# bluenote-1577/sylph

Hardware: AMD Instinct MI355X
Metric: read Gbp/s sketched + genome-comparisons/s profiled, 1 Gbp vs GTDB-R220 (higher is better)
Workload: dtype u64

## Files before the change

sylph_amd/csrc/reads.hip:

```cpp
#include <cstddef>

#include "common.h"
#include "device_common.h"
#include "reads_block.h"
#include "seed_plan.h"
#include "sketch_session.h"

namespace sylph {

namespace {

__global__ __launch_bounds__(256) void block_records_kernel(const uint64_t* __restrict__ off, uint64_t n_rec, uint32_t bias,
                                                            uint32_t rt, uint32_t n_entries, uint32_t* __restrict__ blk_rec,
                                                            uint32_t* __restrict__ count_sentinel, uint32_t* __restrict__ state_words) {
    const uint32_t b = blockIdx.x * blockDim.x + threadIdx.x;
    if (b == 0) { *count_sentinel = 0; state_words[0] = 0; state_words[1] = 0; }
    if (b >= n_entries) return;
    blk_rec[b] = (uint32_t)first_record_of_block(off, n_rec, bias, b, rt);
}

#ifndef SYLPH_READS_HASH_DEFAULT
#define SYLPH_READS_HASH_DEFAULT 1
#endif
#ifndef SYLPH_READS_WAVES
#define SYLPH_READS_WAVES 5
#endif
template <int K, int HV, int ENC, int TPB>
__global__ __launch_bounds__(TPB) __attribute__((amdgpu_waves_per_eu(TPB == 256 ? SYLPH_READS_WAVES : 6, TPB == 256 ? SYLPH_READS_WAVES : 6))) void reads_kernel(const uint8_t* __restrict__ bases_al, uint32_t bias, uint64_t n_al,
                                                     const uint64_t* __restrict__ off, uint64_t n_rec,
                                                     const uint32_t* __restrict__ blk_rec, uint32_t n_blk, uint32_t it_begin, uint32_t it_end,
                                                     uint32_t rt, uint64_t thr,
                                                     uint32_t cand_slack, int avx2_compat, int paired, int want_markers, uint64_t rec_base,
                                                     uint32_t slot_cap, OccRec* __restrict__ slot_rec,
                                                     uint32_t* __restrict__ slot_key, int key_sh,
                                                     uint32_t* __restrict__ blk_count,
                                                     ReadsState* __restrict__ state, const uint32_t* __restrict__ blk_list,
                                                     uint32_t* __restrict__ spill_slot_of_blk) {
    const ReadsLds<TPB> s = reads_lds<TPB>();
    const uint32_t tid = threadIdx.x;
    const uint64_t thr_loop = HV == 2 ? (uint64_t)((uint32_t)(thr >> 32) + 1u + cand_slack) : thr;
    if (tid == 0) *s.redo = 0;
    const uint32_t n_words = stream_words(rt), per_xcd = xcd_share(n_blk);
    for (uint32_t it0 = it_begin + blockIdx.x; it0 < it_end; it0 += gridDim.x) {
        const uint32_t it = blk_list ? it0 : xcd_deal_share(it0, per_xcd);
        if (it >= n_blk) continue;
        const uint32_t blk = blk_list ? blk_list[it] : it;
        const int64_t a0 = block_a0(blk, rt);
        load_stream<ENC, TPB>(s.sF, bases_al, n_al, a0, n_words);
        const uint64_t R0 = blk_rec[blk], R1 = blk_rec[blk + 1];
        const uint64_t w_lo = paired ? (R0 & ~1ull) : R0;
        const bool in_lds = stage_offsets(s, off, n_rec, R0, R1, w_lo);
        __syncthreads();
        uint32_t base_prev = 0;
        const uint64_t out0 = (uint64_t)it * slot_cap;
        for (uint64_t pass = R0; pass < R1; pass += TPB) {
            uint64_t L, s1, s2, e2;
            uint32_t nh, rel;
            if (record_geometry<K>(s, off, in_lds, w_lo, pass + tid, R1, paired, bias, a0, avx2_compat, L, s1, s2, e2, nh, rel))
                state->long_record = 1u;
            uint32_t slot, rel_h, nh_h, rows;
            const bool dealt = deal_by_length(s, nh, rel, slot, rel_h, nh_h, rows);
            hash_record<K, HV>(s, slot, rel_h, nh_h, thr_loop);
            if (dealt) __syncthreads();
            uint32_t total = 0;
            for (;;) {
                uint32_t first;
                const uint32_t cnt = count_hits(s, nh, first, total);
                publish_markers(s, cnt, first, total, want_markers, paired, L, s1, s2, e2, rel, bias, a0);
                const bool is_listed = list_survivors(s, nh, cnt, first, total, rows);
                __syncthreads();
                finish_survivors<K, HV>(s, is_listed, rows, total, base_prev, slot_cap, thr, rec_base, pass, paired, avx2_compat, out0, slot_rec,
                                        slot_key, key_sh);
                __syncthreads();
                if constexpr (HV != 2) break;
                else {
                    if (!*s.redo) break;
                    __syncthreads();
                    if (tid == 0) *s.redo = 0;
                }
            }
            base_prev += total;
        }
        if (tid == 0) close_slots(blk_list != nullptr, blk, it, base_prev, slot_cap, blk_count, &state->spill, spill_slot_of_blk);
        __syncthreads();
    }
}

__global__ __launch_bounds__(64) void compact_occ_kernel(const OccRec* __restrict__ slot_rec, const uint32_t* __restrict__ blk_count,
                                                         const uint32_t* __restrict__ blk_off, uint32_t n_blk, uint32_t slot_cap,
                                                         uint32_t spill_cap, const OccRec* __restrict__ spill_rec,
                                                         const uint32_t* __restrict__ spill_slot_of_blk,
                                                         uint64_t* __restrict__ out_hash, OccRec* __restrict__ out_rec) {
    for (uint32_t b = blockIdx.x; b < n_blk; b += gridDim.x) {
        const uint32_t n = blk_count[b], d = blk_off[b];
        const OccRec* sr = slot_rec + (uint64_t)b * slot_cap;
        if (n > slot_cap) sr = spill_rec + (uint64_t)spill_slot_of_blk[b] * spill_cap;
        for (uint32_t i = threadIdx.x; i < n; i += blockDim.x) {
            const OccRec r = sr[i];
            out_hash[d + i] = r.hash;
            out_rec[d + i] = r;
        }
    }
}

uint32_t grid_for(uint64_t n, uint32_t tpb = 256) { return (uint32_t)((n + tpb - 1) / tpb); }

__global__ __launch_bounds__(1024) void block_total_kernel(const uint32_t* __restrict__ blk_count, uint32_t n_blk, uint32_t* __restrict__ total) {
    __shared__ uint32_t s[16];
    uint32_t v = 0;
    for (uint32_t i = threadIdx.x; i < n_blk; i += 1024) v += blk_count[i];
#pragma unroll
    for (int d = 32; d > 0; d >>= 1) v += (uint32_t)__shfl_xor((int)v, d);
    if ((threadIdx.x & 63) == 0) s[threadIdx.x >> 6] = v;
    __syncthreads();
    if (threadIdx.x == 0) {
        uint32_t t = 0;
        for (int w = 0; w < 16; w++) t += s[w];
        *total = t;
    }
}

void compact_region(sylph_sketch* sk, uint32_t n_blk, uint32_t slot_cap, uint32_t n, uint32_t spill_cap, const OccRec* spill_rec) {
    sylph_ctx* ctx = sk->ctx;
    const SlotMeta m = slot_meta_of(sk, n_blk);
    exclusive_sum_u32(ctx, m.blk_count, m.blk_off, (size_t)n_blk + 1);
    const uint64_t need = sk->n_occ + n;
    sk->hash.grow_keep(need * 8, sk->n_occ * 8, ctx->stream);
    sk->recs.grow_keep(need * sizeof(OccRec), sk->n_occ * sizeof(OccRec), ctx->stream);
    {
        ScopedKernelTimer t(ctx, "compact");
        hipLaunchKernelGGL(compact_occ_kernel, dim3(std::min<uint32_t>(n_blk, 1u << 16)), dim3(64), 0, ctx->stream,
                           sk->slot_rec.as<OccRec>(), m.blk_count, m.blk_off, n_blk, slot_cap, spill_cap, spill_rec, m.spill_slot,
                           sk->hash.as<uint64_t>() + sk->n_occ, sk->recs.as<OccRec>() + sk->n_occ);
        SY_HIP(hipGetLastError());
    }
    sk->n_occ = need;
}

}

void resolve_deferred_slots(sylph_sketch* sk) {
    if (!sk->pend.live || !sk->pend.deferred) return;
    sylph_ctx* ctx = sk->ctx;
    const SlotMeta m = slot_meta_of(sk, sk->pend.n_blk);
    hipLaunchKernelGGL(block_total_kernel, dim3(1), dim3(1024), 0, ctx->stream, m.blk_count, sk->pend.n_blk, m.blk_off + sk->pend.n_blk);
    uint32_t res[3] = {0, 0, 0};
    ctx->read_back(res, m.blk_off + sk->pend.n_blk, 12);
    if (res[1] || res[2]) { redo_deferred_batch(sk); return; }
    sk->pend.deferred = false;
    sk->pend.n = res[0];
    if (res[0] == 0) sk->pend = PendingSlots{};
}

void flush_pending_slots(sylph_sketch* sk) {
    resolve_deferred_slots(sk);
    if (!sk->pend.live) return;
    compact_region(sk, sk->pend.n_blk, sk->pend.slot_cap, sk->pend.n, 0, nullptr);
    sk->pend = PendingSlots{};
}

bool push_short_reads(sylph_sketch* sk, const uint8_t* d_bases, uint32_t phase, const uint64_t* d_off, uint64_t n_records, uint64_t n_bases,
                      int enc) {
    sylph_ctx* ctx = sk->ctx;
    const uint32_t bias = enc == SYLPH_ENC_2BIT ? (uint32_t)((uintptr_t)d_bases & 15) * 4u + phase : (uint32_t)((uintptr_t)d_bases & 15);
    const uint8_t* bases_al = d_bases - ((uintptr_t)d_bases & 15);
    const uint64_t n_al = n_bases + bias;
    static const int env_ragged_tpb = [] { const char* e = getenv("SYLPH_HIP_READS_RAGGED_TPB"); return e ? atoi(e) : RTPB; }();
    const ReadsBlockPlan plan = reads_block_plan(n_bases, n_records, bias, sk->c, sk->k, env_ragged_tpb == RTPB_RAGGED);
    const int tpb = plan.tpb;
    const uint32_t rt = plan.rt, n_blk = plan.n_blk, spill_cap = plan.spill_cap, slot_cap = plan.slot_cap;
    const size_t lds_bytes = plan.lds_bytes;
    const uint64_t thr = UINT64_MAX / (uint64_t)sk->c;
    sk->slot_rec.reserve((size_t)n_blk * slot_cap * sizeof(OccRec));
    sk->slot_key.reserve((size_t)n_blk * slot_cap * 4);
    sk->slot_meta.reserve(SlotMeta::bytes(n_blk, sizeof(ReadsState)));
    const SlotMeta m = slot_meta_of(sk, n_blk);
    ReadsState* const state = reinterpret_cast<ReadsState*>(m.state_words);
    static_assert(offsetof(ReadsState, long_record) == 0 && offsetof(ReadsState, spill) == 4 && offsetof(SpillState, n_tiles) == 0,
                  "long_record and spill.n_tiles are the first two words");
    int cus = 256;
    (void)hipDeviceGetAttribute(&cus, hipDeviceAttributeMultiprocessorCount, ctx->device);
    const int hv_want = ctx->reads_hash >= 0 ? ctx->reads_hash : hash_variant_env(SYLPH_READS_HASH_DEFAULT);
    const uint32_t slack = ctx->reads_slack;
    const int hv = (hv_want == 2 && ((thr >> 32) + 1ull + slack) > 0xFFFFFFFFull) ? 1 : hv_want;
    const int key_sh = key_shift(sk->c);
    auto launch = [&](uint32_t n_it, uint32_t it_b, uint32_t it_e, uint32_t cap, OccRec* sr, uint32_t* skey, const uint32_t* list) {
        if (it_e <= it_b) return;
        const uint32_t grid = ctx->reads_wg_per_cu ? (uint32_t)std::min<uint64_t>(it_e - it_b, (uint64_t)cus * ctx->reads_wg_per_cu) : it_e - it_b;
        auto go = [&](auto kc, auto hc, auto ec, auto tc) {
            constexpr int KK = decltype(kc)::value, HH = decltype(hc)::value, EE = decltype(ec)::value, TT = decltype(tc)::value;
            hipLaunchKernelGGL((reads_kernel<KK, HH, EE, TT>), dim3(grid), dim3(TT), lds_bytes, ctx->stream, bases_al, bias, n_al, d_off, n_records,
                               m.blk_rec, n_it, it_b, it_e, rt, thr, slack, sk->avx2_compat, sk->paired, sk->no_dedup ? 0 : 1, sk->rec_base, cap, sr, skey,
                               key_sh, m.blk_count, state, list, m.spill_slot);
        };
        auto with_tpb = [&](auto kc, auto hc, auto ec) {
            if (tpb == RTPB_RAGGED) go(kc, hc, ec, std::integral_constant<int, RTPB_RAGGED>{}); else go(kc, hc, ec, std::integral_constant<int, RTPB>{});
        };
        if (enc == SYLPH_ENC_2BIT) with_k_hv<1, 2>(sk->k, hv, [&](auto kc, auto hc) { with_tpb(kc, hc, std::integral_constant<int, 1>{}); });
        else with_k_hv<0, 2>(sk->k, hv, [&](auto kc, auto hc) { with_tpb(kc, hc, std::integral_constant<int, 0>{}); });
        SY_HIP(hipGetLastError());
    };
    {
        HostPhase ph(ctx, "push: reads kernel");
        {
            ScopedKernelTimer t(ctx, "annotate");
            hipLaunchKernelGGL(block_records_kernel, dim3(grid_for(n_blk + 1)), dim3(256), 0, ctx->stream, d_off, n_records, bias, rt,
                               n_blk + 1, m.blk_rec, m.blk_count + n_blk, m.state_words);
        }
        ctx->seed_gate();
        {
            const uint32_t n_round = xcd_positions(n_blk);
            const uint32_t cut = xcd_tail_cut(n_blk, ctx->turn.done && !ctx->turn.recorded ? ctx->reads_tail_pct : 0);
            {
                ScopedKernelTimer t(ctx, "seeds");
                launch(n_blk, 0, cut, slot_cap, sk->slot_rec.as<OccRec>(), sk->slot_key.as<uint32_t>(), nullptr);
            }
            ctx->seed_done();
            if (cut < n_round) {
                ScopedKernelTimer t(ctx, "seeds");
                launch(n_blk, cut, n_round, slot_cap, sk->slot_rec.as<OccRec>(), sk->slot_key.as<uint32_t>(), nullptr);
            }
        }
        const uint64_t n_expect = plan.n_expect;
        if (sk->borrow_until_finish && sk->n_occ == 0 && sk->rec_base == 0 && ctx->finish_mode == 0 && sk->c >= 2 && n_expect >= 4096 &&
            (uint64_t)n_blk * slot_cap < (1ull << 31)) {
            sk->pend = PendingSlots{};
            sk->pend.live = true;
            sk->pend.deferred = true;
            sk->pend.n_blk = n_blk;
            sk->pend.slot_cap = slot_cap;
            sk->pend.n = n_blk * slot_cap;
            sk->pend.n_expect = (uint32_t)std::min<uint64_t>(n_expect, sk->pend.n);
            sk->pend.bases = d_bases; sk->pend.phase = phase; sk->pend.off = d_off;
            sk->pend.n_records = n_records; sk->pend.n_bases = n_bases; sk->pend.enc = enc;
            if (ctx->profile) ctx->stats["deferred"].launches++;
            return true;
        }
        hipLaunchKernelGGL(block_total_kernel, dim3(1), dim3(1024), 0, ctx->stream, m.blk_count, n_blk, m.blk_off + n_blk);
    }
    uint32_t res[3] = {0, 0, 0};
    SY_HIP(hipMemcpyAsync(ctx->pinned, m.blk_off + n_blk, 12, hipMemcpyDeviceToHost, ctx->stream));
    SY_HIP(hipStreamSynchronize(ctx->stream));
    memcpy(res, ctx->pinned, 12);
    if (!ctx->pending.empty()) profile_collect(ctx);
    if (res[1] || res[2] > SPILL_MAX_TILES) return false;
    const uint32_t n = res[0];
    if (n == 0) return true;
    if (res[2] == 0 && sk->n_occ == 0 && ctx->finish_mode != 1 && sk->c >= 2) {
        sk->pend.live = true;
        sk->pend.n_blk = n_blk;
        sk->pend.slot_cap = slot_cap;
        sk->pend.n = n;
        return true;
    }
    const OccRec* sp_r = nullptr;
    if (res[2]) {
        DevBuf& b_x = ctx->scratch[7];
        b_x.reserve((size_t)res[2] * spill_cap * sizeof(OccRec));
        OccRec* xr = b_x.as<OccRec>();
        ScopedKernelTimer ts(ctx, "seeds_spill");
        ScopedKernelTimer t(ctx, "seeds");
        launch(res[2], 0, res[2], spill_cap, xr, nullptr, state->spill.tiles);
        sp_r = xr;
    }
    compact_region(sk, n_blk, slot_cap, n, spill_cap, sp_r);
    return true;
}

}
```

sylph_amd/csrc/reads_block.h:

```cpp
#pragma once
#include "common.h"
#include "device_common.h"
#include "seed_plan.h"
#include "sketch_session.h"

namespace sylph {
namespace {

using namespace seed_plan;

template <int K>
struct KC {
    static constexpr uint64_t MASK = (1ull << (2 * K)) - 1;
};

#define SY_LDS __attribute__((address_space(3)))
template <int TPB>
struct ReadsLds {
    SY_LDS uint32_t* sF;
    SY_LDS uint64_t* off;
    SY_LDS uint64_t *m0, *m1;
    SY_LDS uint32_t (*mask)[TPB];
    SY_LDS uint32_t* wave;
    SY_LDS uint32_t* first;
    SY_LDS uint32_t* hist;
    SY_LDS uint32_t* rel;
    SY_LDS uint16_t *perm, *nh;
    SY_LDS uint32_t *redo, *redo_deal;
};
template <int TPB>
__device__ __forceinline__ ReadsLds<TPB> reads_lds() {
    constexpr int OFFS = offs_staged(TPB);
    extern __shared__ uint32_t sF[];
    __shared__ uint64_t s_off[OFFS + 4];
    __shared__ uint32_t s_mask[MASKW][TPB];
    __shared__ uint32_t s_wave[TPB / 64];
    __shared__ uint32_t s_first[TPB + 1], s_rel[TPB];
    __shared__ uint16_t s_perm[TPB], s_nh[TPB];
    __shared__ uint32_t s_redo, s_redo_deal;
    static_assert((OFFS + 4) >= 2 * TPB, "the marker arrays alias the staged offsets");
    static_assert(TPB + 1 >= 64, "the histogram aliases s_first");
    using W = SY_LDS uint32_t*; using D = SY_LDS uint64_t*; using H = SY_LDS uint16_t*;
    return ReadsLds<TPB>{(W)sF, (D)s_off, (D)s_off, (D)s_off + TPB, (SY_LDS uint32_t(*)[TPB])s_mask, (W)s_wave, (W)s_first, (W)s_first, (W)s_rel,
                         (H)s_perm, (H)s_nh, (W)&s_redo, (W)&s_redo_deal};
}

__device__ __forceinline__ uint64_t win64(const SY_LDS uint32_t* sF, uint32_t b) {
    const uint32_t j = b >> 4, ph = (b & 15u) * 2u;
    const uint64_t x = ((uint64_t)sF[j] << 32) | sF[j + 1];
    return (x << ph) | ((uint64_t)sF[j + 2] >> (32u - ph));
}

template <int K>
__device__ __forceinline__ uint64_t revcomp_top(uint64_t x) {
    const uint64_t rev = __brevll(x);
    const uint64_t y = ((rev & 0x5555555555555555ull) << 1) | ((rev >> 1) & 0x5555555555555555ull);
    return (~y) & KC<K>::MASK;
}

__device__ __forceinline__ uint32_t even_fields_to_bytes31(uint32_t w) {
    uint32_t t = w & 0xCCCCCCCCu;
    t = (t | (t << 2)) & 0xF0F0F0F0u;
    return t | (t << 4);
}
__device__ __forceinline__ void evenodd16(uint64_t x, uint32_t& ev, uint32_t& od) {
    const uint32_t hi = (uint32_t)(x >> 32), lo = (uint32_t)x;
    ev = __builtin_amdgcn_perm(even_fields_to_bytes31(hi), even_fields_to_bytes31(lo), 0x07050301u);
    od = __builtin_amdgcn_perm(even_fields_to_bytes31(hi << 2), even_fields_to_bytes31(lo << 2), 0x07050301u);
}

template <int K, int T, int HV>
__device__ __forceinline__ void kmer_step(uint32_t A0, uint32_t A1, uint32_t A2, uint32_t B0, uint32_t B1, uint32_t B2,
                                          uint64_t thr, uint32_t& mask) {
    static_assert(2 * K <= 62 && 2 * K > 32, "min_u62 wants both windows below 2^62; the high word holds 2K - 32 bits");
    constexpr int HB = 2 * K - 32, T0 = T & ~1;
    uint32_t fhi, rhi;
    if constexpr (2 * T + HB <= 32) {
        fhi = __builtin_amdgcn_ubfe(A0, 32 - HB - 2 * T, HB); rhi = __builtin_amdgcn_ubfe(B1, 2 * T, HB);
    } else {
        const uint32_t cf = fword<2 * T0>(A0, A1, A2), cr = rword<2 * T0 + 32>(B0, B1, B2);
        fhi = __builtin_amdgcn_ubfe(cf, 32 - HB - 2 * (T - T0), HB); rhi = __builtin_amdgcn_ubfe(cr, 2 * (T - T0), HB);
    }
    const uint32_t flo = fword<2 * T + HB>(A0, A1, A2), rlo = rword<2 * T>(B0, B1, B2);
    const uint64_t canon = min_u62(((uint64_t)fhi << 32) | flo, ((uint64_t)rhi << 32) | rlo);
    if constexpr (HV == 2) {
        const uint32_t u = mm_hash64_gfx950_hi1(canon);
        asm("v_cmp_ge_u32 vcc, %2, %1\n\tv_addc_co_u32 %0, vcc, %0, %0, vcc" : "+v"(mask) : "v"(u), "s"((uint32_t)thr) : "vcc");
    } else {
        const uint64_t h = HV ? mm_hash64_gfx950(canon) : mm_hash64(canon);
        asm("v_cmp_lt_u64 vcc, %1, %2\n\tv_addc_co_u32 %0, vcc, %0, %0, vcc" : "+v"(mask) : "v"(h), "s"(thr) : "vcc");
    }
}
template <int K, int T0, int HV>
__device__ __forceinline__ void kmer_steps8(uint32_t A0, uint32_t A1, uint32_t A2, uint32_t B0, uint32_t B1, uint32_t B2,
                                            uint64_t thr, uint32_t& mask) {
    kmer_step<K, T0 + 0, HV>(A0, A1, A2, B0, B1, B2, thr, mask);
    kmer_step<K, T0 + 1, HV>(A0, A1, A2, B0, B1, B2, thr, mask);
    kmer_step<K, T0 + 2, HV>(A0, A1, A2, B0, B1, B2, thr, mask);
    kmer_step<K, T0 + 3, HV>(A0, A1, A2, B0, B1, B2, thr, mask);
    kmer_step<K, T0 + 4, HV>(A0, A1, A2, B0, B1, B2, thr, mask);
    kmer_step<K, T0 + 5, HV>(A0, A1, A2, B0, B1, B2, thr, mask);
    kmer_step<K, T0 + 6, HV>(A0, A1, A2, B0, B1, B2, thr, mask);
    kmer_step<K, T0 + 7, HV>(A0, A1, A2, B0, B1, B2, thr, mask);
}

template <int ENC, int TPB>
__device__ __forceinline__ void load_stream(SY_LDS uint32_t* sF, const uint8_t* bases_al, uint64_t n_al, int64_t a0, uint32_t n_words) {
    const uint32_t tid = threadIdx.x;
    const bool interior = a0 >= 0 && (uint64_t)(a0 + (int64_t)n_words * 16) <= n_al;
    if (interior) {
        if constexpr (ENC == 0) {
            const uint4* src = reinterpret_cast<const uint4*>(bases_al + a0);
            for (uint32_t ci = tid; ci < n_words; ci += TPB) sF[ci] = pack16_fwd(src[ci]);
        } else {
            const uint32_t* src = reinterpret_cast<const uint32_t*>(bases_al + (a0 >> 2));
            for (uint32_t ci = tid; ci < n_words; ci += TPB) sF[ci] = __builtin_amdgcn_perm(0u, src[ci], 0x00010203u);
        }
    } else {
        for (uint32_t ci = tid; ci < n_words; ci += TPB) {
            const int64_t a = a0 + (int64_t)ci * 16;
            if constexpr (ENC == 0) {
                uint4 v = make_uint4(0, 0, 0, 0);
                if (a >= 0 && (uint64_t)a < n_al) v = *reinterpret_cast<const uint4*>(bases_al + a);
                sF[ci] = pack16_fwd(v);
            } else {
                uint32_t w = 0;
                if (a >= 0 && (uint64_t)a < n_al) w = *reinterpret_cast<const uint32_t*>(bases_al + (a >> 2));
                sF[ci] = __builtin_amdgcn_perm(0u, w, 0x00010203u);
            }
        }
    }
}

template <int TPB>
__device__ __forceinline__ bool stage_offsets(const ReadsLds<TPB> s, const uint64_t* off, uint64_t n_rec, uint64_t R0, uint64_t R1,
                                              uint64_t w_lo) {
    const uint64_t w_hi = min(R1 + 2, n_rec);
    const bool in_lds = (w_hi - w_lo + 1) <= (uint64_t)(offs_staged(TPB) + 4) && (R1 - R0) <= (uint64_t)TPB;
    if (in_lds)
        for (uint64_t t = threadIdx.x; t <= w_hi - w_lo; t += TPB) s.off[t] = off[w_lo + t];
    return in_lds;
}

template <int K, int TPB>
__device__ __forceinline__ bool record_geometry(const ReadsLds<TPB> s, const uint64_t* off, bool in_lds, uint64_t w_lo, uint64_t r,
                                                uint64_t R1, int paired, uint32_t bias, int64_t a0, int avx2_compat, uint64_t& L,
                                                uint64_t& s1, uint64_t& s2, uint64_t& e2, uint32_t& nh, uint32_t& rel) {
    const bool active = r < R1;
    uint64_t start = 0;
    L = 0; s1 = 0; s2 = 0; e2 = 0;
    if (active) {
        if (in_lds) {
            start = s.off[r - w_lo];
            L = s.off[r + 1 - w_lo] - start;
            if (paired) { const uint64_t r1 = (r & ~1ull) - w_lo; s1 = s.off[r1]; s2 = s.off[r1 + 1]; e2 = s.off[r1 + 2]; }
        } else {
            start = off[r];
            L = off[r + 1] - start;
            if (paired) { const uint64_t r1 = r & ~1ull; s1 = off[r1]; s2 = off[r1 + 1]; e2 = off[r1 + 2]; }
        }
    }
    const bool too_long = active && (L > (uint64_t)RH || (paired && (s2 - s1 > (uint64_t)RH || e2 - s2 > (uint64_t)RH)));
    nh = (active && !too_long) ? (uint32_t)n_hashed_kmers(L, K, avx2_compat, 0) : 0u;
    rel = active ? record_rel(start, bias, a0) : 0u;
    return too_long;
}

template <int TPB>
__device__ __forceinline__ bool deal_by_length(const ReadsLds<TPB> s, uint32_t nh, uint32_t rel, uint32_t& slot, uint32_t& rel_h, uint32_t& nh_h,
                                               uint32_t& rows) {
    const uint32_t tid = threadIdx.x, lane = tid & 63;
    if (tid < 64) s.hist[tid] = 0;
    s.rel[tid] = rel;
    s.nh[tid] = (uint16_t)nh;
    if (tid == 0) *s.redo_deal = 0;
    __syncthreads();
    if (__ballot(nh != (uint32_t)s.nh[0]) && lane == 0) *s.redo_deal = 1;
    __syncthreads();
    const bool dealt = *s.redo_deal != 0;
    const uint32_t bin = deal_bin(nh);
    uint32_t hg_max = half_groups(nh), arrival = 0, hc = 0;
    if (dealt) {
        arrival = atomicAdd((uint32_t*)&s.hist[bin], 1u);
        __syncthreads();
        hc = s.hist[lane];
        const uint64_t bins_used = __ballot(hc != 0u);
        hg_max = bins_used ? 63u - (uint32_t)(__ffsll((unsigned long long)bins_used) - 1) : 0u;
    }
    rows = rows_used(hg_max);
    if (dealt) {
        const uint32_t incl = wave_inclusive_sum(hc);
        s.perm[(uint32_t)__shfl((int)(incl - hc), (int)bin) + arrival] = (uint16_t)tid;
        __syncthreads();
    }
    slot = dealt ? s.perm[tid] : tid;
    rel_h = dealt ? s.rel[slot] : rel;
    nh_h = dealt ? s.nh[slot] : nh;
    return dealt;
}

template <int K, int HV, int TPB>
__device__ __forceinline__ void hash_record(const ReadsLds<TPB> s, uint32_t slot, uint32_t rel_h, uint32_t nh_h, uint64_t thr_loop) {
    const SY_LDS uint32_t* const sF = s.sF;
    uint32_t nh_max = nh_h;
#pragma unroll
    for (int d = 32; d > 0; d >>= 1) nh_max = max(nh_max, (uint32_t)__shfl_xor((int)nh_max, d));
    if (nh_max) {
        const uint32_t w0 = rel_h >> 4, sh = 32u - (rel_h & 15u) * 2u;
        uint32_t raw = sF[w0], nxt = sF[w0 + 1];
        auto next_word = [&](uint32_t j) {
            const uint32_t a = (uint32_t)((((uint64_t)raw << 32) | nxt) >> sh);
            raw = nxt;
            nxt = sF[w0 + j + 2];
            return a;
        };
        uint32_t A0 = next_word(0), A1 = next_word(1), A2 = next_word(2);
        uint32_t B0 = rcword(A0), B1 = rcword(A1), B2 = rcword(A2);
        const uint32_t n_half = half_groups(nh_max);
        SY_LDS uint16_t* const mask_half = (SY_LDS uint16_t*)&s.mask[0][slot];
        const uint32_t n_grp = n_half >> 1;
        for (uint32_t g = 0; g < n_grp; g++) {
            uint32_t mask = 0;
            kmer_steps8<K, 0, HV>(A0, A1, A2, B0, B1, B2, thr_loop, mask);
            kmer_steps8<K, 8, HV>(A0, A1, A2, B0, B1, B2, thr_loop, mask);
            A0 = A1; A1 = A2; A2 = next_word(g + 3);
            B0 = B1; B1 = B2; B2 = rcword(A2);
            mask_half[group_half(g, TPB)] = (uint16_t)mask;
        }
        if (n_half & 1u) {
            uint32_t mask = 0;
            kmer_steps8<K, 0, HV>(A0, A1, A2, B0, B1, B2, thr_loop, mask);
            mask_half[group_half(n_grp, TPB)] = (uint16_t)(mask << 8);
        }
    }
}

template <int TPB>
__device__ __forceinline__ uint32_t count_hits(const ReadsLds<TPB> s, uint32_t nh, uint32_t& first, uint32_t& total) {
    const uint32_t tid = threadIdx.x;
    uint32_t cnt = 0;
    const uint32_t nw = mask_words(nh);
    for (uint32_t w = 0; w + 1 < nw; w++) cnt += __popc(s.mask[w][tid]);
    if (nw) {
        const uint32_t m = s.mask[nw - 1][tid] & tail_mask(nh);
        s.mask[nw - 1][tid] = m;
        cnt += __popc(m);
    }
    first = block_excl_sum<TPB>(cnt, (uint32_t*)s.wave, &total);
    return cnt;
}

template <int TPB>
__device__ __forceinline__ void publish_markers(const ReadsLds<TPB> s, uint32_t cnt, uint32_t first, uint32_t total, int want_markers, int paired,
                                                uint64_t L, uint64_t s1, uint64_t s2, uint64_t e2, uint32_t rel, uint32_t bias, int64_t a0) {
    const uint32_t tid = threadIdx.x;
    uint64_t m0 = 0, m1 = 0;
    uint32_t has = 0;
    if (cnt && want_markers) {
        uint32_t ba = 0, bb = 0;
        if (!paired) {
            if (L >= 66 && L <= 400) { has = 1; ba = rel; bb = rel + (uint32_t)(L / 2); }
        } else if (s2 - s1 >= 33 && e2 - s2 >= 33) {
            has = 1;
            ba = record_rel(s1, bias, a0);
            bb = record_rel(s2, bias, a0);
        }
        if (has) {
            const uint64_t wa64 = win64(s.sF, ba), wb64 = win64(s.sF, bb);
            uint32_t ea, oa, eb, ob;
            evenodd16(wa64, ea, oa);
            evenodd16(wb64, eb, ob);
            m0 = (uint64_t)ea | ((uint64_t)eb << 32);
            m1 = (uint64_t)oa | ((uint64_t)ob << 32);
        }
    }
    s.m0[tid] = m0;
    s.m1[tid] = m1;
    s.first[tid] = first | (has << 31);
    if (tid == 0) s.first[TPB] = total;
}

template <int TPB>
__device__ __forceinline__ bool list_survivors(const ReadsLds<TPB> s, uint32_t nh, uint32_t cnt, uint32_t first, uint32_t total, uint32_t rows) {
    const uint32_t tid = threadIdx.x;
    SY_LDS uint32_t* const s_owner = &s.mask[0][0] + rows * TPB;
    const bool is_listed = listed(total, rows, TPB);
    if (is_listed && cnt) {
        uint32_t p = first;
        for (uint32_t w = 0; w < mask_words(nh); w++) {
            uint32_t m = s.mask[w][tid];
            while (m) {
                const uint32_t bpos = (uint32_t)__clz((int)m);
                s_owner[p++] = tid | ((w * 32 + bpos) << OWNER_LANE_BITS);
                m &= ~(0x80000000u >> bpos);
            }
        }
    }
    return is_listed;
}

template <int K, int HV, int TPB>
__device__ __forceinline__ void finish_survivors(const ReadsLds<TPB> s, bool is_listed, uint32_t rows, uint32_t total, uint32_t base_prev,
                                                 uint32_t slot_cap, uint64_t thr, uint64_t rec_base, uint64_t pass, int paired, int avx2_compat,
                                                 uint64_t out0, OccRec* slot_rec, uint32_t* slot_key, int key_sh) {
    const SY_LDS uint32_t* const s_owner = &s.mask[0][0] + rows * TPB;
    for (uint32_t hix = threadIdx.x; hix < total; hix += TPB) {
        uint32_t lo, i = 0, f;
        if (is_listed) {
            const uint32_t ow = s_owner[hix];
            lo = ow & ((1u << OWNER_LANE_BITS) - 1u);
            i = ow >> OWNER_LANE_BITS;
            f = s.first[lo];
        } else {
            lo = 0;
            uint32_t hi = TPB;
            while (hi - lo > 1) {
                const uint32_t mid = (lo + hi) >> 1;
                if ((s.first[mid] & 0x7FFFFFFFu) <= hix) lo = mid; else hi = mid;
            }
            f = s.first[lo];
            uint32_t j = hix - (f & 0x7FFFFFFFu);
            for (uint32_t w = 0; w < MASKW; w++) {
                uint32_t m = s.mask[w][lo];
                const uint32_t c = (uint32_t)__popc(m);
                if (j >= c) { j -= c; continue; }
                for (; j; j--) m &= ~(0x80000000u >> __clz((int)m));
                i = w * 32 + (uint32_t)__clz((int)m);
                break;
            }
        }
        const uint32_t o = base_prev + hix;
        if (o < slot_cap) {
            const uint64_t ft = win64(s.sF, s.rel[lo] + i);
            const uint64_t fk = ft >> (64 - 2 * K), rk = revcomp_top<K>(ft);
            const uint64_t h = mm_hash64_gfx950(fk < rk ? fk : rk);
            if constexpr (HV == 2) {
                if (h >= thr) {
                    atomicAnd((uint32_t*)&s.mask[kmer_word(i)][lo], ~(1u << kmer_bit(i)));
                    *s.redo = 1u;
                    continue;
                }
            }
            uint64_t rid = rec_base + pass + lo;
            if (f >> 31) {
                rid |= RID_MARKER_BIT;
                if (paired) rid |= min(emission_rank(i, s.nh[lo], avx2_compat), RID_RANK_MAX) << RID_RANK_SHIFT;
            }
            slot_rec[out0 + o] = OccRec{h, rid, s.m0[lo], s.m1[lo]};
            if (slot_key) slot_key[out0 + o] = (uint32_t)(h >> key_sh);
        }
    }
}

#undef SY_LDS

}
}
```

sylph_amd/csrc/seed_plan.h:

```cpp
#pragma once
#include <cstddef>
#include <cstdint>

#if defined(__HIPCC__)
#define SY_SEED_HD __host__ __device__ __forceinline__
#else
#define SY_SEED_HD inline
#endif

namespace sylph {
namespace seed_plan {

constexpr int RTPB = 256;
constexpr int RTPB_RAGGED = 512;
constexpr int RT_MIN = 4096, RT_MAX = 65536;
constexpr int RH = 400;
constexpr int K_MIN = 21;
constexpr int NH_MAX = RH - (K_MIN - 1);
constexpr int RPAD = 32;
constexpr int MASKW = 12;
constexpr int OFFS_256 = 600;
SY_SEED_HD constexpr int offs_staged(int tpb) { return tpb == RTPB ? OFFS_256 : 2 * tpb + 80; }
constexpr int OWNER_LANE_BITS = 10;

constexpr int TPB = 256;
constexpr int WPT = 4;
constexpr int TILE_WORDS = TPB * WPT;
constexpr int TILE_BASES = TILE_WORDS * 16;
constexpr int HALO_WORDS = 2;
constexpr int STAGE_CAP = 1024;
constexpr int FLUSH_AT = 512;
constexpr int LIST_CAP = 2048;

SY_SEED_HD constexpr uint32_t half_groups(uint32_t nh) { return (nh + 7u) >> 3; }

SY_SEED_HD constexpr uint32_t slot_capacity(uint64_t full, uint64_t expect) {
    const uint64_t want = expect + expect * 3 / 4 + 48;
    return (uint32_t)(full < want ? full : want);
}

SY_SEED_HD constexpr int64_t block_a0(uint32_t blk, uint32_t rt) { return (int64_t)blk * rt - RH; }
SY_SEED_HD constexpr uint32_t stream_words(uint32_t rt) { return (rt + 2u * RH) / 16u + 3u; }
SY_SEED_HD constexpr uint32_t lds_words(uint32_t rt) { return stream_words(rt) + RPAD; }
SY_SEED_HD constexpr uint64_t block_begin(uint32_t blk, uint32_t rt) { return (uint64_t)blk * rt; }
SY_SEED_HD uint64_t first_record_of_block(const uint64_t* off, uint64_t n_rec, uint32_t bias, uint32_t blk, uint32_t rt) {
    const uint64_t target = block_begin(blk, rt);
    uint64_t lo = 0, hi = n_rec;
    while (lo < hi) {
        const uint64_t mid = (lo + hi) >> 1;
        if (off[mid] + bias < target) lo = mid + 1; else hi = mid;
    }
    return lo;
}
SY_SEED_HD constexpr uint32_t record_rel(uint64_t start, uint32_t bias, int64_t a0) { return (uint32_t)((int64_t)(start + bias) - a0); }
SY_SEED_HD constexpr uint32_t hash_hi_word(uint32_t rel, uint32_t nh_max) { return (rel >> 4) + 4u + (half_groups(nh_max) >> 1); }
SY_SEED_HD constexpr uint32_t win64_hi_word(uint32_t b) { return (b >> 4) + 2u; }

SY_SEED_HD constexpr uint32_t kmer_word(uint32_t i) { return i >> 5; }
SY_SEED_HD constexpr uint32_t kmer_bit(uint32_t i) { return 31u - (i & 31u); }
SY_SEED_HD constexpr uint32_t group_half(uint32_t g, uint32_t tpb) { return ((g >> 1) * tpb * 2u) + ((g & 1u) ^ 1u); }
SY_SEED_HD constexpr uint32_t mask_words(uint32_t nh) { return (nh + 31u) >> 5; }
SY_SEED_HD constexpr uint32_t tail_mask(uint32_t nh) { return (uint32_t)(0xFFFFFFFF00000000ull >> (nh - (mask_words(nh) - 1u) * 32u)); }
SY_SEED_HD constexpr uint32_t rows_used(uint32_t hg_max) { const uint32_t r = (hg_max * 8u + 31u) >> 5; return r < (uint32_t)MASKW ? r : (uint32_t)MASKW; }
SY_SEED_HD constexpr bool listed(uint32_t total, uint32_t rows, uint32_t tpb) { return total <= ((uint32_t)MASKW - rows) * tpb; }
SY_SEED_HD constexpr uint32_t deal_bin(uint32_t nh) { return 63u - half_groups(nh); }

SY_SEED_HD constexpr uint32_t xcd_share(uint32_t n) { return (n + 7u) / 8u; }
SY_SEED_HD constexpr uint32_t xcd_deal_share(uint32_t i, uint32_t share) { return (i & 7u) * share + (i >> 3); }
SY_SEED_HD constexpr uint32_t xcd_deal(uint32_t i, uint32_t n) { return xcd_deal_share(i, xcd_share(n)); }
SY_SEED_HD constexpr uint32_t xcd_positions(uint32_t n) { return xcd_share(n) * 8u; }
SY_SEED_HD constexpr uint32_t xcd_tail_cut(uint32_t n, uint32_t tail_pct) {
    const uint32_t n_round = xcd_positions(n);
    return (tail_pct && n_round >= 64u) ? (uint32_t)((uint64_t)n_round * (100u - tail_pct) / 100u) & ~7u : n_round;
}

struct ReadsBlockPlan {
    int tpb;
    uint32_t rt;
    uint32_t n_blk;
    uint32_t slot_cap;
    uint32_t spill_cap;
    size_t lds_bytes;
    uint64_t n_expect;
};
inline ReadsBlockPlan reads_block_plan(uint64_t n_bases, uint64_t n_records, uint32_t bias, uint32_t c, uint32_t k, bool ragged_tpb_wanted) {
    ReadsBlockPlan p{};
    const bool ragged = (n_bases % n_records) != 0;
    p.tpb = (ragged && ragged_tpb_wanted && (uint64_t)RTPB_RAGGED * 93 / 100 * n_bases / n_records <= (uint64_t)RT_MAX) ? RTPB_RAGGED : RTPB;
    const uint64_t target = ragged ? (uint64_t)p.tpb * 93 / 100 : (uint64_t)p.tpb;
    const uint64_t want = target * n_bases / n_records;
    p.rt = (uint32_t)(want < (uint64_t)RT_MIN ? RT_MIN : want > (uint64_t)RT_MAX ? RT_MAX : want);
    p.rt = (p.rt + 15u) & ~15u;
    p.n_blk = (uint32_t)((n_bases + bias) / p.rt) + 1;
    p.spill_cap = p.rt + RH;
    p.slot_cap = slot_capacity(p.spill_cap, (uint64_t)p.rt / c);
    p.lds_bytes = (size_t)lds_words(p.rt) * 4;
    p.n_expect = (n_bases > n_records * (uint64_t)(k - 1) ? n_bases - n_records * (uint64_t)(k - 1) : 0) / c;
    return p;
}

struct SlotMeta {
    uint32_t *blk_rec, *blk_count, *spill_slot, *blk_off, *state_words;
    SlotMeta(uint32_t* base, uint32_t n_blk)
        : blk_rec(base), blk_count(blk_rec + (n_blk + 1)), spill_slot(blk_count + (n_blk + 1)), blk_off(spill_slot + (n_blk + 1)),
          state_words(blk_off + (n_blk + 1)) {}
    static size_t bytes(uint32_t n_blk, size_t state_bytes) { return ((size_t)n_blk + 1) * 4 * 4 + state_bytes + 16; }
};

static_assert(RT_MIN % 16 == 0 && RT_MAX % 16 == 0 && RT_MIN <= RT_MAX && RH % 16 == 0, "blocks and halo are whole 16-base words");
static_assert(MASKW * 32 >= NH_MAX, "a record's k-mers have a mask bit each");
static_assert(half_groups(NH_MAX) <= 63 && deal_bin(NH_MAX) < 64 && deal_bin(0) == 63, "63 bins hold the half-groups of the longest record");
static_assert(RTPB_RAGGED <= (1 << OWNER_LANE_BITS) && (uint64_t)MASKW * 32 <= (1ull << (32 - OWNER_LANE_BITS)), "the owner word tid | idx << 10 holds 512 lanes and MASKW * 32 indices");
static_assert(RTPB % 64 == 0 && RTPB_RAGGED % 64 == 0 && RTPB <= RTPB_RAGGED, "whole wavefronts");
static_assert(offs_staged(RTPB) + 4 >= 2 * RTPB && offs_staged(RTPB_RAGGED) + 4 >= 2 * RTPB_RAGGED, "the marker arrays alias the staged offsets");
static_assert(hash_hi_word(RH + RT_MIN - 1, NH_MAX) < lds_words(RT_MIN) && hash_hi_word(RH + RT_MAX - 1, NH_MAX) < lds_words(RT_MAX), "RPAD covers the idle lanes' reads");
static_assert(win64_hi_word(RH + RT_MAX - 1 + RH - 1) < stream_words(RT_MAX) && win64_hi_word(RH + RT_MIN - 1 + RH - 1) < stream_words(RT_MIN), "every window of a record or its mate is loaded");
static_assert((((TILE_WORDS + HALO_WORDS - 1) << 4) | 15) < (1 << 16), "the 16-bit descriptor (word << 4) | off holds TILE_WORDS + HALO_WORDS");
static_assert((TPB - 1) * WPT + 6 <= TILE_WORDS + HALO_WORDS && WPT + HALO_WORDS == 6, "a lane's six words end inside TILE_WORDS + HALO_WORDS");
static_assert(HALO_WORDS * 16 >= 31 && HALO_WORDS <= TPB, "the halo holds the k - 1 bases behind the tile");
static_assert(FLUSH_AT <= STAGE_CAP && LIST_CAP <= TILE_BASES && LIST_CAP <= (1 << 16), "staging and list sizes");
static_assert(slot_capacity(TILE_BASES, TILE_BASES) == TILE_BASES, "a tile never gets more slots than positions");

}
}
```

Baseline: 1211.

## Record k-mer hits with predicated LDS xor instead of register mask accumulation

For the default block size, each k-mer hash comparison now sets exec by compare and issues a ds_xor_b32 of a per-position bit constant directly into the LDS mask column, instead of shifting the result into a register mask and storing halves. Columns are zeroed beforehand and the lower half is periodically cleared, with a decode step (m ^ m<<16) applied on the first count pass. This is meant to shorten the per-k-mer dependency chain on the mask register, at the cost of many extra LDS atomic-like writes, exec manipulation in inline asm, extra zeroing work and a decode pass.

```diff
diff --git a/sylph_amd/csrc/reads.hip b/sylph_amd/csrc/reads.hip
--- a/sylph_amd/csrc/reads.hip
+++ b/sylph_amd/csrc/reads.hip
@@ -25,6 +25,8 @@
 #ifndef SYLPH_READS_WAVES
 #define SYLPH_READS_WAVES 5
 #endif
+template <int TPB>
+constexpr bool hit_bits_by_lds = TPB == RTPB;
 template <int K, int HV, int ENC, int TPB>
 __global__ __launch_bounds__(TPB) __attribute__((amdgpu_waves_per_eu(TPB == 256 ? SYLPH_READS_WAVES : 6, TPB == 256 ? SYLPH_READS_WAVES : 6))) void reads_kernel(const uint8_t* __restrict__ bases_al, uint32_t bias, uint64_t n_al,
                                                      const uint64_t* __restrict__ off, uint64_t n_rec,
@@ -40,6 +42,7 @@
     const uint32_t tid = threadIdx.x;
     const uint64_t thr_loop = HV == 2 ? (uint64_t)((uint32_t)(thr >> 32) + 1u + cand_slack) : thr;
     if (tid == 0) *s.redo = 0;
+    const HitRegs hit = hit_bits_by_lds<TPB> ? hit_regs() : HitRegs{};
     const uint32_t n_words = stream_words(rt), per_xcd = xcd_share(n_blk);
     for (uint32_t it0 = it_begin + blockIdx.x; it0 < it_end; it0 += gridDim.x) {
         const uint32_t it = blk_list ? it0 : xcd_deal_share(it0, per_xcd);
@@ -59,13 +62,15 @@
             if (record_geometry<K>(s, off, in_lds, w_lo, pass + tid, R1, paired, bias, a0, avx2_compat, L, s1, s2, e2, nh, rel))
                 state->long_record = 1u;
             uint32_t slot, rel_h, nh_h, rows;
-            const bool dealt = deal_by_length(s, nh, rel, slot, rel_h, nh_h, rows);
-            hash_record<K, HV>(s, slot, rel_h, nh_h, thr_loop);
+            const bool dealt = deal_by_length<TPB, hit_bits_by_lds<TPB>>(s, nh, rel, slot, rel_h, nh_h, rows);
+            hash_record<K, HV, TPB, hit_bits_by_lds<TPB>>(s, slot, rel_h, nh_h, thr_loop, hit);
             if (dealt) __syncthreads();
             uint32_t total = 0;
+            bool decode = hit_bits_by_lds<TPB>;
             for (;;) {
                 uint32_t first;
-                const uint32_t cnt = count_hits(s, nh, first, total);
+                const uint32_t cnt = count_hits(s, nh, decode, first, total);
+                decode = false;
                 publish_markers(s, cnt, first, total, want_markers, paired, L, s1, s2, e2, rel, bias, a0);
                 const bool is_listed = list_survivors(s, nh, cnt, first, total, rows);
                 __syncthreads();
diff --git a/sylph_amd/csrc/reads_block.h b/sylph_amd/csrc/reads_block.h
--- a/sylph_amd/csrc/reads_block.h
+++ b/sylph_amd/csrc/reads_block.h
@@ -69,9 +69,26 @@
     od = __builtin_amdgcn_perm(even_fields_to_bytes31(hi << 2), even_fields_to_bytes31(lo << 2), 0x07050301u);
 }
 
-template <int K, int T, int HV>
+struct HitRegs {
+    uint32_t bit[16];
+    uint32_t zero;
+    uint64_t exec0;
+};
+__device__ __forceinline__ HitRegs hit_regs() {
+    HitRegs r;
+#pragma unroll
+    for (int t = 0; t < 16; t++) asm("v_mov_b32 %0, %1" : "=v"(r.bit[t]) : "s"(hit_const(t)));
+    asm("v_mov_b32 %0, 0" : "=v"(r.zero));
+    r.exec0 = 0;
+    return r;
+}
+__device__ __forceinline__ void hit_clear_lower(uint32_t& addr, uint32_t zero) { asm("ds_write_b16 %0, %1" : "+v"(addr) : "v"(zero)); }
+__device__ __forceinline__ void hit_chain_begin(uint32_t& addr) { asm volatile("" : "+v"(addr) : : "memory"); }
+__device__ __forceinline__ void hit_chain_end(uint32_t& addr) { asm volatile("s_waitcnt lgkmcnt(0)" : "+v"(addr) : : "memory"); }
+
+template <int K, int T, int HV, bool LB>
 __device__ __forceinline__ void kmer_step(uint32_t A0, uint32_t A1, uint32_t A2, uint32_t B0, uint32_t B1, uint32_t B2,
-                                          uint64_t thr, uint32_t& mask) {
+                                          uint64_t thr, uint32_t& mask, const HitRegs& hit) {
     static_assert(2 * K <= 62 && 2 * K > 32, "min_u62 wants both windows below 2^62; the high word holds 2K - 32 bits");
     constexpr int HB = 2 * K - 32, T0 = T & ~1;
     uint32_t fhi, rhi;
@@ -85,23 +102,31 @@
     const uint64_t canon = min_u62(((uint64_t)fhi << 32) | flo, ((uint64_t)rhi << 32) | rlo);
     if constexpr (HV == 2) {
         const uint32_t u = mm_hash64_gfx950_hi1(canon);
-        asm("v_cmp_ge_u32 vcc, %2, %1\n\tv_addc_co_u32 %0, vcc, %0, %0, vcc" : "+v"(mask) : "v"(u), "s"((uint32_t)thr) : "vcc");
+        if constexpr (LB)
+            asm("v_cmpx_ge_u32 vcc, %2, %1\n\tds_xor_b32 %0, %3\n\ts_mov_b64 exec, %4"
+                : "+v"(mask) : "v"(u), "s"((uint32_t)thr), "v"(hit.bit[T]), "s"(hit.exec0) : "vcc");
+        else
+            asm("v_cmp_ge_u32 vcc, %2, %1\n\tv_addc_co_u32 %0, vcc, %0, %0, vcc" : "+v"(mask) : "v"(u), "s"((uint32_t)thr) : "vcc");
     } else {
         const uint64_t h = HV ? mm_hash64_gfx950(canon) : mm_hash64(canon);
-        asm("v_cmp_lt_u64 vcc, %1, %2\n\tv_addc_co_u32 %0, vcc, %0, %0, vcc" : "+v"(mask) : "v"(h), "s"(thr) : "vcc");
-    }
-}
-template <int K, int T0, int HV>
+        if constexpr (LB)
+            asm("v_cmpx_lt_u64 vcc, %1, %2\n\tds_xor_b32 %0, %3\n\ts_mov_b64 exec, %4"
+                : "+v"(mask) : "v"(h), "s"(thr), "v"(hit.bit[T]), "s"(hit.exec0) : "vcc");
+        else
+            asm("v_cmp_lt_u64 vcc, %1, %2\n\tv_addc_co_u32 %0, vcc, %0, %0, vcc" : "+v"(mask) : "v"(h), "s"(thr) : "vcc");
+    }
+}
+template <int K, int T0, int HV, bool LB>
 __device__ __forceinline__ void kmer_steps8(uint32_t A0, uint32_t A1, uint32_t A2, uint32_t B0, uint32_t B1, uint32_t B2,
-                                            uint64_t thr, uint32_t& mask) {
-    kmer_step<K, T0 + 0, HV>(A0, A1, A2, B0, B1, B2, thr, mask);
-    kmer_step<K, T0 + 1, HV>(A0, A1, A2, B0, B1, B2, thr, mask);
-    kmer_step<K, T0 + 2, HV>(A0, A1, A2, B0, B1, B2, thr, mask);
-    kmer_step<K, T0 + 3, HV>(A0, A1, A2, B0, B1, B2, thr, mask);
-    kmer_step<K, T0 + 4, HV>(A0, A1, A2, B0, B1, B2, thr, mask);
-    kmer_step<K, T0 + 5, HV>(A0, A1, A2, B0, B1, B2, thr, mask);
-    kmer_step<K, T0 + 6, HV>(A0, A1, A2, B0, B1, B2, thr, mask);
-    kmer_step<K, T0 + 7, HV>(A0, A1, A2, B0, B1, B2, thr, mask);
+                                            uint64_t thr, uint32_t& mask, const HitRegs& hit) {
+    kmer_step<K, T0 + 0, HV, LB>(A0, A1, A2, B0, B1, B2, thr, mask, hit);
+    kmer_step<K, T0 + 1, HV, LB>(A0, A1, A2, B0, B1, B2, thr, mask, hit);
+    kmer_step<K, T0 + 2, HV, LB>(A0, A1, A2, B0, B1, B2, thr, mask, hit);
+    kmer_step<K, T0 + 3, HV, LB>(A0, A1, A2, B0, B1, B2, thr, mask, hit);
+    kmer_step<K, T0 + 4, HV, LB>(A0, A1, A2, B0, B1, B2, thr, mask, hit);
+    kmer_step<K, T0 + 5, HV, LB>(A0, A1, A2, B0, B1, B2, thr, mask, hit);
+    kmer_step<K, T0 + 6, HV, LB>(A0, A1, A2, B0, B1, B2, thr, mask, hit);
+    kmer_step<K, T0 + 7, HV, LB>(A0, A1, A2, B0, B1, B2, thr, mask, hit);
 }
 
 template <int ENC, int TPB>
@@ -166,7 +191,7 @@
     return too_long;
 }
 
-template <int TPB>
+template <int TPB, bool LB>
 __device__ __forceinline__ bool deal_by_length(const ReadsLds<TPB> s, uint32_t nh, uint32_t rel, uint32_t& slot, uint32_t& rel_h, uint32_t& nh_h,
                                                uint32_t& rows) {
     const uint32_t tid = threadIdx.x, lane = tid & 63;
@@ -188,6 +213,10 @@
         hg_max = bins_used ? 63u - (uint32_t)(__ffsll((unsigned long long)bins_used) - 1) : 0u;
     }
     rows = rows_used(hg_max);
+    if constexpr (LB) {
+        const uint32_t rows_u = (uint32_t)__builtin_amdgcn_readfirstlane((int)rows);
+        for (uint32_t w = 0; w < rows_u; w += 2) { s.mask[w][tid] = 0; s.mask[w + 1][tid] = 0; }
+    }
     if (dealt) {
         const uint32_t incl = wave_inclusive_sum(hc);
         s.perm[(uint32_t)__shfl((int)(incl - hc), (int)bin) + arrival] = (uint16_t)tid;
@@ -199,12 +228,14 @@
     return dealt;
 }
 
-template <int K, int HV, int TPB>
-__device__ __forceinline__ void hash_record(const ReadsLds<TPB> s, uint32_t slot, uint32_t rel_h, uint32_t nh_h, uint64_t thr_loop) {
+template <int K, int HV, int TPB, bool LB>
+__device__ __forceinline__ void hash_record(const ReadsLds<TPB> s, uint32_t slot, uint32_t rel_h, uint32_t nh_h, uint64_t thr_loop,
+                                            const HitRegs& hit_consts) {
     const SY_LDS uint32_t* const sF = s.sF;
     uint32_t nh_max = nh_h;
 #pragma unroll
     for (int d = 32; d > 0; d >>= 1) nh_max = max(nh_max, (uint32_t)__shfl_xor((int)nh_max, d));
+    if constexpr (LB) nh_max = (uint32_t)__builtin_amdgcn_readfirstlane((int)nh_max);
     if (nh_max) {
         const uint32_t w0 = rel_h >> 4, sh = 32u - (rel_h & 15u) * 2u;
         uint32_t raw = sF[w0], nxt = sF[w0 + 1];
@@ -219,30 +250,56 @@
         const uint32_t n_half = half_groups(nh_max);
         SY_LDS uint16_t* const mask_half = (SY_LDS uint16_t*)&s.mask[0][slot];
         const uint32_t n_grp = n_half >> 1;
+        if constexpr (LB) {
+            HitRegs hit = hit_consts;
+            hit.exec0 = __builtin_amdgcn_read_exec();
+            uint32_t addr = (uint32_t)(uintptr_t)&s.mask[0][slot];
+            hit_chain_begin(addr);
+            for (uint32_t g = 0; g < n_grp; g++) {
+                kmer_steps8<K, 0, HV, true>(A0, A1, A2, B0, B1, B2, thr_loop, addr, hit);
+                kmer_steps8<K, 8, HV, true>(A0, A1, A2, B0, B1, B2, thr_loop, addr, hit);
+                A0 = A1; A1 = A2; A2 = next_word(g + 3);
+                B0 = B1; B1 = B2; B2 = rcword(A2);
+                if (hit_clear_after(g)) hit_clear_lower(addr, hit.zero);
+                else addr += hit_word_offset(2, TPB);
+            }
+            if (n_half & 1u) {
+                kmer_steps8<K, 0, HV, true>(A0, A1, A2, B0, B1, B2, thr_loop, addr, hit);
+                if (hit_clear_after(n_grp)) hit_clear_lower(addr, hit.zero);
+            }
+            hit_chain_end(addr);
+            return;
+        }
+        const HitRegs hit{};
         for (uint32_t g = 0; g < n_grp; g++) {
             uint32_t mask = 0;
-            kmer_steps8<K, 0, HV>(A0, A1, A2, B0, B1, B2, thr_loop, mask);
-            kmer_steps8<K, 8, HV>(A0, A1, A2, B0, B1, B2, thr_loop, mask);
+            kmer_steps8<K, 0, HV, false>(A0, A1, A2, B0, B1, B2, thr_loop, mask, hit);
+            kmer_steps8<K, 8, HV, false>(A0, A1, A2, B0, B1, B2, thr_loop, mask, hit);
             A0 = A1; A1 = A2; A2 = next_word(g + 3);
             B0 = B1; B1 = B2; B2 = rcword(A2);
             mask_half[group_half(g, TPB)] = (uint16_t)mask;
         }
         if (n_half & 1u) {
             uint32_t mask = 0;
-            kmer_steps8<K, 0, HV>(A0, A1, A2, B0, B1, B2, thr_loop, mask);
+            kmer_steps8<K, 0, HV, false>(A0, A1, A2, B0, B1, B2, thr_loop, mask, hit);
             mask_half[group_half(n_grp, TPB)] = (uint16_t)(mask << 8);
         }
     }
 }
 
 template <int TPB>
-__device__ __forceinline__ uint32_t count_hits(const ReadsLds<TPB> s, uint32_t nh, uint32_t& first, uint32_t& total) {
+__device__ __forceinline__ uint32_t count_hits(const ReadsLds<TPB> s, uint32_t nh, bool decode, uint32_t& first, uint32_t& total) {
     const uint32_t tid = threadIdx.x;
     uint32_t cnt = 0;
     const uint32_t nw = mask_words(nh);
-    for (uint32_t w = 0; w + 1 < nw; w++) cnt += __popc(s.mask[w][tid]);
+    for (uint32_t w = 0; w + 1 < nw; w++) {
+        uint32_t m = s.mask[w][tid];
+        if (decode) { m = hit_decode(m); s.mask[w][tid] = m; }
+        cnt += __popc(m);
+    }
     if (nw) {
-        const uint32_t m = s.mask[nw - 1][tid] & tail_mask(nh);
+        const uint32_t m0 = s.mask[nw - 1][tid];
+        const uint32_t m = (decode ? hit_decode(m0) : m0) & tail_mask(nh);
         s.mask[nw - 1][tid] = m;
         cnt += __popc(m);
     }
diff --git a/sylph_amd/csrc/seed_plan.h b/sylph_amd/csrc/seed_plan.h
--- a/sylph_amd/csrc/seed_plan.h
+++ b/sylph_amd/csrc/seed_plan.h
@@ -65,6 +65,23 @@
 SY_SEED_HD constexpr bool listed(uint32_t total, uint32_t rows, uint32_t tpb) { return total <= ((uint32_t)MASKW - rows) * tpb; }
 SY_SEED_HD constexpr uint32_t deal_bin(uint32_t nh) { return 63u - half_groups(nh); }
 
+SY_SEED_HD constexpr uint32_t hit_const(uint32_t t) { return 0x00010001u << (15u - t); }
+SY_SEED_HD constexpr bool hit_clear_after(uint32_t g) { return (g & 1u) == 0u; }
+SY_SEED_HD constexpr uint32_t hit_cleared(uint32_t m) { return m & 0xFFFF0000u; }
+SY_SEED_HD constexpr uint32_t hit_decode(uint32_t m) { return m ^ (m << 16); }
+SY_SEED_HD constexpr uint32_t hit_word_offset(uint32_t g, uint32_t tpb) { return (g >> 1) * tpb * 4u; }
+inline void hit_encode_model(const uint8_t* hits, uint32_t n_half, uint32_t* col) {
+    for (uint32_t w = 0; w < rows_used(n_half); w++) col[w] = 0;
+    const uint32_t n_grp = n_half >> 1;
+    for (uint32_t g = 0; g < n_grp + (n_half & 1u); g++) {
+        uint32_t& word = col[hit_word_offset(g, 1) / 4u];
+        const uint32_t n_t = g < n_grp ? 16u : 8u;
+        for (uint32_t t = 0; t < n_t; t++)
+            if (hits[g * 16u + t]) word ^= hit_const(t);
+        if (hit_clear_after(g)) word = hit_cleared(word);
+    }
+}
+
 SY_SEED_HD constexpr uint32_t xcd_share(uint32_t n) { return (n + 7u) / 8u; }
 SY_SEED_HD constexpr uint32_t xcd_deal_share(uint32_t i, uint32_t share) { return (i & 7u) * share + (i >> 3); }
 SY_SEED_HD constexpr uint32_t xcd_deal(uint32_t i, uint32_t n) { return xcd_deal_share(i, xcd_share(n)); }
@@ -109,6 +126,7 @@
 
 static_assert(RT_MIN % 16 == 0 && RT_MAX % 16 == 0 && RT_MIN <= RT_MAX && RH % 16 == 0, "blocks and halo are whole 16-base words");
 static_assert(MASKW * 32 >= NH_MAX, "a record's k-mers have a mask bit each");
+static_assert(MASKW % 2 == 0, "the columns are zeroed two rows at a time (deal_by_length)");
 static_assert(half_groups(NH_MAX) <= 63 && deal_bin(NH_MAX) < 64 && deal_bin(0) == 63, "63 bins hold the half-groups of the longest record");
 static_assert(RTPB_RAGGED <= (1 << OWNER_LANE_BITS) && (uint64_t)MASKW * 32 <= (1ull << (32 - OWNER_LANE_BITS)), "the owner word tid | idx << 10 holds 512 lanes and MASKW * 32 indices");
 static_assert(RTPB % 64 == 0 && RTPB_RAGGED % 64 == 0 && RTPB <= RTPB_RAGGED, "whole wavefronts");
```

New measurement: 1229, median of 6. 1.01x the previous value.
